# yzh503/vm-placement-migration-gym

Measured on AMD Instinct MI355X. Metric: env-steps/sec (batched) at 100-PM config, 1/2/4/8 GPUs; reward MAE vs CPU ref, higher is better.
Workload: dtype f64

## Files before the change

vm-placement-migration-gym_amd/csrc/vmp_env_common.h:

```cpp
#ifndef VMP_ENV_COMMON_H
#define VMP_ENV_COMMON_H

#include <hip/hip_runtime.h>
#include <math.h>
#include <stdint.h>

#include "vmp_dev.h"
#include "vmp_kernels.h"
#include "vmp_layout.h"
#include "vmp_np_rng.h"
#include "vmp_np_sort.h"
#include "vmp_np_sum.h"
#include "vmp_stamps.h"

namespace vmp {

struct Lds {
  EnvHdr LDSP *hdr;
  double LDSP *cpu, *mem;
  float LDSP *fcpu, *fmem;
  uint8_t LDSP *tc, *tm;
  uint16_t LDSP *ord;
  uint64_t LDSP *bc;
  int32_t LDSP *sortstk;
  uint16_t LDSP *nulls;
  uint8_t LDSP *accc, *accm;
  double LDSP *jobres;
  int32_t LDSP *arr;
  uint32_t LDSP *svc;
  uint64_t LDSP *svcst;
  uint64_t LDSP *svcfb;
  int32_t LDSP *svcinfo;
  uint8_t LDSP *ccomp, *mcomp;
  uint64_t LDSP *pdirty;
  uint32_t LDSP *evw;
  int32_t LDSP *evt;
  uint8_t LDSP *evok;
  PwLds pw;
  char LDSP *base;
};

__device__ __forceinline__ Lds make_lds(const EnvParams &p, char LDSP *base) {
  Lds L;
  L.hdr = reinterpret_cast<EnvHdr LDSP *>(base + p.off_hdr);
  L.cpu = reinterpret_cast<double LDSP *>(base + p.off_pm);
  L.mem = L.cpu + p.P;
  L.fcpu = reinterpret_cast<float LDSP *>(base + p.off_fpm);
  L.fmem = L.fcpu + p.fmem_off;
  L.tc = reinterpret_cast<uint8_t LDSP *>(base + p.off_thr);
  L.tm = L.tc + p.tm_off;
  L.ord = reinterpret_cast<uint16_t LDSP *>(base + p.off_ord);
  L.bc = reinterpret_cast<uint64_t LDSP *>(base + p.off_bits);
  L.sortstk = reinterpret_cast<int32_t LDSP *>(base + p.off_sort);
  L.nulls = reinterpret_cast<uint16_t LDSP *>(base + p.off_bits);
  L.accc = reinterpret_cast<uint8_t LDSP *>(base + p.off_acc);
  L.accm = L.accc + p.acc_cap;
  L.jobres = reinterpret_cast<double LDSP *>(base + p.off_stage);
  L.svcinfo = reinterpret_cast<int32_t LDSP *>(base + p.off_stage + kStageSvcInfo);
  L.svcfb = reinterpret_cast<uint64_t LDSP *>(base + p.off_stage + kStageSvcFb);
  L.svcst = reinterpret_cast<uint64_t LDSP *>(base + p.off_pre);
  L.svc = reinterpret_cast<uint32_t LDSP *>(base + p.off_pre + kSpecStateBytes * p.scap);
  L.arr = reinterpret_cast<int32_t LDSP *>(base + p.off_pre + kSpecDrawBytes * p.scap);
  L.pdirty = reinterpret_cast<uint64_t LDSP *>(base + p.off_pdirty);
  L.ccomp = reinterpret_cast<uint8_t LDSP *>(base + p.off_ccomp);
  L.mcomp = L.ccomp + p.ccomp_cap;
  L.evw = reinterpret_cast<uint32_t LDSP *>(base + p.off_ev);
  L.evt = reinterpret_cast<int32_t LDSP *>(L.evw + kEvCap);
  L.evok = reinterpret_cast<uint8_t LDSP *>(L.evt + kEvCap);
  L.pw.lo = reinterpret_cast<int32_t LDSP *>(base + p.off_leaf);
  L.pw.len = L.pw.lo + p.n_leaf;
  L.pw.stk = L.pw.len + p.n_leaf;
  L.pw.val = reinterpret_cast<double LDSP *>(base + p.off_leafval);
  L.base = base;
  return L;
}

struct Tables {
  double cent[128];
  float fcent[128];
  PoisConst pois[2];
};
static_assert(sizeof(Tables) == 1696 && sizeof(Tables) <= kEnvStaticLds, "k_env static LDS");

__device__ __forceinline__ int w_pl(uint32_t w) { return (int)(w & 0xFFFFu); }
constexpr int kPad = 0xFFFF;
__device__ __forceinline__ bool live(uint32_t w) { return w_pl(w) != kPad; }
__device__ __forceinline__ int w_cc(uint32_t w) { return (int)((w >> 16) & 0xFFu); }
__device__ __forceinline__ int w_cm(uint32_t w) { return (int)(w >> 24); }
__device__ __forceinline__ uint32_t w_make(int pl, int cc, int cm) {
  return (uint32_t)pl | ((uint32_t)cc << 16) | ((uint32_t)cm << 24);
}

__device__ __forceinline__ Pcg ld_pcg(const EnvHdr LDSP *h, int k) {
  Pcg r;
  r.s = U128{h->rng[k][0], h->rng[k][1]};
  r.inc = U128{h->rng[k][2], h->rng[k][3]};
  return r;
}
__device__ __forceinline__ void st_pcg(EnvHdr LDSP *h, int k, const Pcg &r) {
  if (lane_id() == 0) {
    h->rng[k][0] = r.s.hi;
    h->rng[k][1] = r.s.lo;
  }
}

__device__ __forceinline__ float fcent_of(int k) { return (float)((double)k * 0.01); }

__device__ __forceinline__ int fit_threshold(float f) {
  int k0 = (int)((1.0f - f) * 100.0f);
  k0 = k0 < 0 ? 0 : (k0 > 100 ? 100 : k0);
  const bool up = k0 < 100 && f + fcent_of(k0 + 1) <= 1.0f;
  const bool at = f + fcent_of(k0) <= 1.0f;
  return up ? k0 + 1 : (at ? k0 : k0 - 1);
}

__device__ __forceinline__ uint32_t prefix_or32(uint32_t x) {
  x |= (uint32_t)__builtin_amdgcn_update_dpp(0, (int)x, 0x111, 0xF, 0xF, false);
  x |= (uint32_t)__builtin_amdgcn_update_dpp(0, (int)x, 0x112, 0xF, 0xF, false);
  x |= (uint32_t)__builtin_amdgcn_update_dpp(0, (int)x, 0x114, 0xF, 0xF, false);
  x |= (uint32_t)__builtin_amdgcn_update_dpp(0, (int)x, 0x118, 0xF, 0xF, false);
  x |= (uint32_t)__builtin_amdgcn_update_dpp(0, (int)x, 0x142, 0xA, 0xF, false);
  x |= (uint32_t)__builtin_amdgcn_update_dpp(0, (int)x, 0x143, 0xC, 0xF, false);
  return x;
}
__device__ __forceinline__ uint64_t prefix_or64(uint64_t x) {
  return ((uint64_t)prefix_or32((uint32_t)(x >> 32)) << 32) | prefix_or32((uint32_t)x);
}

__device__ __forceinline__ uint32_t prefix_max32(uint32_t x) {
  x = max(x, (uint32_t)__builtin_amdgcn_update_dpp(0, (int)x, 0x111, 0xF, 0xF, false));
  x = max(x, (uint32_t)__builtin_amdgcn_update_dpp(0, (int)x, 0x112, 0xF, 0xF, false));
  x = max(x, (uint32_t)__builtin_amdgcn_update_dpp(0, (int)x, 0x114, 0xF, 0xF, false));
  x = max(x, (uint32_t)__builtin_amdgcn_update_dpp(0, (int)x, 0x118, 0xF, 0xF, false));
  x = max(x, (uint32_t)__builtin_amdgcn_update_dpp(0, (int)x, 0x142, 0xA, 0xF, false));
  x = max(x, (uint32_t)__builtin_amdgcn_update_dpp(0, (int)x, 0x143, 0xC, 0xF, false));
  return x;
}

__device__ __forceinline__ uint64_t readlane_u64(uint64_t x, int l) {
  const uint32_t lo = (uint32_t)__builtin_amdgcn_readlane((int)(uint32_t)x, l);
  const uint32_t hi = (uint32_t)__builtin_amdgcn_readlane((int)(uint32_t)(x >> 32), l);
  return ((uint64_t)hi << 32) | lo;
}

__device__ __forceinline__ void build_fitmax(const EnvParams &p, const Lds &L, uint32_t LDSP *M) {
  const int lane = lane_id();
  M[lane] = 0;
  M[lane + 64] = 0;
  wsync();
  for (int q = lane; q < p.P; q += 64) {
    const int tcq = (int)L.tc[q];
    if (tcq > 0) __atomic_fetch_max(&M[tcq - 1], (uint32_t)L.tm[q], __ATOMIC_RELAXED);
  }
  wsync();
  const int rlo = 63 - lane, rhi = 127 - lane;
  const bool hi_ok = rhi <= 100;
  uint32_t c1 = hi_ok ? M[rhi] : 0u, c0 = M[rlo];
  c1 = prefix_max32(c1);
  c0 = max(prefix_max32(c0), (uint32_t)__builtin_amdgcn_readlane((int)c1, 63));
  wsync();
  M[rlo] = c0;
  if (hi_ok) M[rhi] = c1;
  wsync();
}

__device__ __forceinline__ int ff_scan(const EnvParams &p, const Lds &L, int kc, int km) {
  const int lane = lane_id();
  for (int b = 0; b < p.P; b += 64) {
    const int i = b + lane;
    const bool f = i < p.P && (int)L.tc[i] - 1 >= kc && (int)L.tm[i] - 1 >= km;
    const uint64_t m = ballot(f);
    if (m) return b + __ffsll((unsigned long long)m) - 1;
  }
  return -1;
}

__device__ __forceinline__ int bf_tie(const EnvParams &p, const Lds &L, int kc, int km, int above,
                                   int eq);
__device__ __forceinline__ int bf_choose(const EnvParams &p, const Lds &L, int kc, int km) {
  const int lane = lane_id();
  const int P = p.P;
  float best = -INFINITY;
  int cnt = 0, bi = -1;
  for (int i = lane; i < P; i += 64) {
    if ((int)L.tc[i] - 1 >= kc && (int)L.tm[i] - 1 >= km) {
      const float key = L.fcpu[i] + L.fmem[i];
      if (key > best) {
        best = key;
        cnt = 1;
        bi = i;
      } else if (key == best) {
        cnt++;
      }
    }
  }
  float m = best;
#pragma unroll
  for (int o = 32; o > 0; o >>= 1) m = fmaxf(m, __shfl_xor(m, o));
  int tot = (best == m) ? cnt : 0;
#pragma unroll
  for (int o = 32; o > 0; o >>= 1) tot += __shfl_xor(tot, o);
  if (tot == 0) return -1;
  if (tot == 1) {
    const uint64_t who = ballot(best == m && cnt == 1);
    return __builtin_amdgcn_readlane(bi, __ffsll((unsigned long long)who) - 1);
  }
  int above = 0, eq = 0;
  for (int i = lane; i < P; i += 64) {
    const float key = L.fcpu[i] + L.fmem[i];
    above += key > m;
    eq += key == m;
  }
#pragma unroll
  for (int o = 32; o > 0; o >>= 1) {
    above += __shfl_xor(above, o);
    eq += __shfl_xor(eq, o);
  }
  return bf_tie(p, L, kc, km, above, eq);
}

__device__ __forceinline__ int bf_tie(const EnvParams &p, const Lds &L, int kc, int km, int above,
                                   int eq) {
  const int lane = lane_id();
  const int P = p.P;
  for (int i = lane; i < P; i += 64) L.ord[i] = (uint16_t)i;
  const int hi = P - above - 1, lo = P - above - eq;
  wsync();
  const uint8_t LDSP *tc = L.tc, *tm = L.tm;
  const int pos = wave_aqselect_top(
      KeySum{L.fcpu, L.fmem}, L.ord, P, L.sortstk, lo, hi,
      reinterpret_cast<uint16_t LDSP *>(L.sortstk + kSortStackWords),
      [=](int q) { return (int)tc[q] - 1 >= kc && (int)tm[q] - 1 >= km; });
  return pos >= 0 ? (int)L.ord[pos] : -1;
}

__device__ __forceinline__ void mark_pm(const Lds &L, int P, int q) {
  L.pdirty[q >> 6] |= 1ull << (q & 63);
  L.pdirty[(P + q) >> 6] |= 1ull << ((P + q) & 63);
}

__device__ __forceinline__ bool env_place(const Lds &L, const Tables &T, int P, int q, int kc,
                                          int km) {
  double cq = L.cpu[q], mq = L.mem[q];
  double vc = T.cent[kc], vm = T.cent[km];
  bool ok = (cq + vc <= 1) && (mq + vm <= 1);
  wsync();
  if (ok && lane_id() == 0) {
    L.cpu[q] = cq + vc;
    L.mem[q] = mq + vm;
    mark_pm(L, P, q);
  }
  wsync();
  return ok;
}

__device__ __noinline__ uint32_t svc_fallback(uint64_t LDSP *st, const uint64_t LDSP *inc,
                                              const PoisConst *c) {
  Pcg r;
  r.s = U128{st[0], st[1]};
  r.inc = U128{inc[0], inc[1]};
  const int64_t x = poisson(r, *c);
  __builtin_amdgcn_fence(__ATOMIC_SEQ_CST, "wavefront");
  __builtin_amdgcn_wave_barrier();
  if ((threadIdx.x & 63) == 0) {
    st[0] = r.s.hi;
    st[1] = r.s.lo;
  }
  __builtin_amdgcn_fence(__ATOMIC_SEQ_CST, "wavefront");
  __builtin_amdgcn_wave_barrier();
  return (uint32_t)(x + 1);
}

struct ParRng {
  U128 base, inc;
  U128 st;
  double u;
  int pos;
};
__device__ __forceinline__ U128 rl128(U128 x, int l) {
  return U128{readlane_u64(x.hi, l), readlane_u64(x.lo, l)};
}
__device__ __forceinline__ void par_fill(ParRng &g, const U128 &JA, const U128 &JM) {
  g.st = add128(mul128(JA, g.base), mul128(JM, g.inc));
  const uint64_t x = g.st.hi ^ g.st.lo;
  const unsigned rot = (unsigned)(g.st.hi >> 58);
  const uint64_t out = (x >> rot) | (x << ((64 - rot) & 63));
  g.u = (double)(out >> 11) * (1.0 / 9007199254740992.0);
  g.pos = 0;
}
__device__ __forceinline__ void par_next_chunk(ParRng &g, const U128 &JA, const U128 &JM) {
  g.base = rl128(g.st, 63);
  par_fill(g, JA, JM);
}
__device__ __forceinline__ U128 par_state(const ParRng &g) {
  return g.pos == 0 ? g.base : rl128(g.st, uni(g.pos - 1));
}

__device__ __forceinline__ int64_t par_poisson_mult(ParRng &g, double enlam, const U128 &JA,
                                                    const U128 &JM) {
  double prod = 1.0;
  int64_t X = 0;
#pragma unroll 1
  for (;;) {
    if (g.pos == 64) par_next_chunk(g, JA, JM);
    prod *= readlane_f64(g.u, uni(g.pos));
    g.pos++;
    if (prod > enlam)
      X += 1;
    else
      return X;
  }
}

struct PtrsChunk {
  uint64_t acc;
  int64_t k;
  bool valid;
};
__device__ __forceinline__ void par_ptrs_eval(const ParRng &g, const PoisConst &c, PtrsChunk &pc) {
  const int lane = lane_id();
  const int i = lane & 31;
  const double U = __shfl(g.u, 2 * i) - 0.5;
  const double V = __shfl(g.u, 2 * i + 1);
  const double us = 0.5 - fabs(U);
  const int64_t k = (int64_t)floor((2 * c.a / us + c.b) * U + c.lam + 0.43);
  bool ok;
  if ((us >= 0.07) && (V <= c.vr))
    ok = true;
  else if ((k < 0) || ((us < 0.013) && (V > us)))
    ok = false;
  else
    ok = ptrs_accept(V, us, k, c.lam, c.a, c.b, c.loglam, c.log_invalpha, c.loggam_tab, c.tab_n);
  pc.acc = ballot(ok && lane < 32);
  pc.k = k;
  pc.valid = true;
}
__device__ __forceinline__ int64_t par_poisson_ptrs(ParRng &g, const PoisConst &c, PtrsChunk &pc,
                                                    const U128 &JA, const U128 &JM) {
#pragma unroll 1
  for (;;) {
    if (g.pos == 64) {
      par_next_chunk(g, JA, JM);
      pc.valid = false;
    }
    if (!pc.valid) par_ptrs_eval(g, c, pc);
    const uint64_t m = pc.acc & (~0ull << (g.pos >> 1));
    if (m == 0) {
      g.pos = 64;
      continue;
    }
    const int i = uni(__builtin_ctzll(m));
    g.pos = 2 * i + 2;
    return (int64_t)readlane_u64((uint64_t)pc.k, i);
  }
}

__device__ __forceinline__ int64_t par_poisson(ParRng &g, const PoisConst &c, PtrsChunk &pc,
                                               const U128 &JA, const U128 &JM) {
  if (c.kind == 0) return 0;
  if (c.kind == 1) return par_poisson_mult(g, c.enlam, JA, JM);
  return par_poisson_ptrs(g, c, pc, JA, JM);
}

__device__ __forceinline__ void predraw(const EnvParams &p, const Lds &L, const Tables &T,
                                        int K, int V, const U128 &JA, const U128 &JM) {
  const int lane = lane_id();
  EnvHdr LDSP *H = L.hdr;
  ParRng g;
  PtrsChunk pc;
  pc.valid = false;
  Pcg r3 = ld_pcg(H, 2);
  g.base = r3.s;
  g.inc = r3.inc;
  par_fill(g, JA, JM);
  int64_t need = 0;
#pragma unroll 1
  for (int k = 0; k < K; k++) {
    const int64_t a = par_poisson(g, T.pois[0], pc, JA, JM);
    if (lane == 0) L.arr[k] = (int32_t)(a < 0x7fffffff ? a : 0x7fffffff);
    need += a < V ? a : V;
  }
  r3.s = par_state(g);
  st_pcg(H, 2, r3);
  Pcg r4 = ld_pcg(H, 3);
  const uint64_t hint = H->pad;
  const bool none_free = K == 1 && (hint >> 63) && ((hint >> 32) & 1u) == 0 &&
                         (uint32_t)hint > (uint32_t)H->timestep + 1u;
  const int S = none_free ? 0 : (int)(need < p.scap ? need : p.scap);
  g.base = r4.s;
  g.inc = r4.inc;
  pc.valid = false;
  if (S > 0) par_fill(g, JA, JM);
#pragma unroll 1
  for (int j = 0; j < S; j++) {
    const int64_t x = par_poisson(g, T.pois[1], pc, JA, JM);
    const U128 sj = par_state(g);
    if (lane == 0) {
      L.svc[j] = (uint32_t)(x + 1);
      L.svcst[2 * j] = sj.hi;
      L.svcst[2 * j + 1] = sj.lo;
    }
  }
  const U128 fb = S > 0 ? par_state(g) : r4.s;
  if (lane == 0) {
    L.svcfb[0] = fb.hi;
    L.svcfb[1] = fb.lo;
    L.svcinfo[0] = S;
    L.svcinfo[1] = 0;
  }
  wsync();
}

constexpr int kSrcConfig = 0, kSrcEnv = 1, kSrcTrace = 2;
template <int SRC>
__device__ __forceinline__ const PoisConst *env_pois(const EnvParams &p, int e) {
  return SRC == kSrcEnv ? p.pois + 2 * (int64_t)e : p.pois;
}

template <int SRC>
__device__ __forceinline__ uint32_t svc_take(const EnvParams &p, const Lds &L, int e) {
  const int S = L.svcinfo[0], used = L.svcinfo[1];
  uint32_t x;
  if (used < S) {
    x = L.svc[used];
  } else {
    x = svc_fallback(L.svcfb, &L.hdr->rng[3][2], env_pois<SRC>(p, e) + 1);
  }
  wsync();
  if (lane_id() == 0) L.svcinfo[1] = used + 1;
  wsync();
  return x;
}

__device__ __forceinline__ void svc_commit(const Lds &L) {
  const int S = L.svcinfo[0], used = L.svcinfo[1];
  if (used == 0) return;
  uint64_t hi, lo;
  if (used <= S) {
    hi = L.svcst[2 * (used - 1)];
    lo = L.svcst[2 * (used - 1) + 1];
  } else {
// ... 60 lines not shown
```

vm-placement-migration-gym_amd/csrc/vmp_env_wave.h:

```cpp
#ifndef VMP_ENV_WAVE_H
#define VMP_ENV_WAVE_H

#include <hip/hip_runtime.h>
#include <stdint.h>

#include "vmp_dev.h"
#include "vmp_env_common.h"
#include "vmp_kernels.h"
#include "vmp_launch_order.h"
#include "vmp_layout.h"
#include "vmp_stamps.h"

namespace vmp {

template <int VPT>
__device__ __forceinline__ int64_t heuristic_apply(const EnvParams &p, const Lds &L,
                                                   const Tables &T, uint32_t (&wa)[VPT],
                                                   int policy, int32_t *act_out,
                                                   uint8_t *valid_out, bool quiet, int qkind,
                                                   bool &fit_any STAMP_PARAMS) {
  const int lane = lane_id();
  const int P = p.P, WAIT = p.P;
  const bool bf = policy == 1;
  uint32_t pend = 0;
#pragma unroll
  for (int s = 0; s < VPT; s++)
    if (w_pl(wa[s]) == WAIT) pend |= 1u << s;
  uint32_t won = 0, bad = 0;
  int64_t n_place = 0;
  fit_any = false;
#ifdef VMP_CHECK_QUIET
  if (ballot(pend != 0)) {
#else
  if (!quiet && ballot(pend != 0)) {
#endif
    for (int i = lane; i < P; i += 64) {
      const float fcv = (float)L.cpu[i], fmv = (float)L.mem[i];
      L.fcpu[i] = fcv;
      L.fmem[i] = fmv;
      L.tc[i] = (uint8_t)(fit_threshold(fcv) + 1);
      L.tm[i] = (uint8_t)(fit_threshold(fmv) + 1);
    }
    wsync();
    STAMP(16);
    uint32_t hit = 0;
    uint32_t LDSP *M = reinterpret_cast<uint32_t LDSP *>(L.bc);
    build_fitmax(p, L, M);
#pragma unroll
    for (int s = 0; s < VPT; s++)
      hit |= (uint32_t)(((pend >> s) & 1u) && M[w_cc(wa[s])] > (uint32_t)w_cm(wa[s])) << s;
    const bool anyfit = ballot(hit != 0) != 0;
    fit_any = anyfit;
#ifdef VMP_CHECK_QUIET
    if (quiet && qkind == 1 && anyfit && lane == 0)
      __hip_atomic_fetch_add(gptr(&g_quiet_violations), 1ull, __ATOMIC_RELAXED,
                             __HIP_MEMORY_SCOPE_AGENT);
#endif
    STAMP(17);
#pragma unroll 1
    for (; anyfit;) {
      const int mine = hit ? (__builtin_ctz(hit) << 6) | lane : 2047;
      const int best = 2047 - (int)__builtin_amdgcn_readlane(
                                  (int)prefix_max32((uint32_t)(2047 - mine)), 63);
      STAMP(18);
      if (best == 2047) break;
      const int ws = best >> 6, wl = best & 63;
      uint32_t own = 0;
#pragma unroll
      for (int s = 0; s < VPT; s++)
        if (s == ws) own = wa[s];
      const uint32_t ww = rdlane(own, wl);
#pragma unroll
      for (int s = 0; s < VPT; s++)
        if (s < ws || (s == ws && lane <= wl)) pend &= ~(1u << s);
      hit &= pend;
      const int kc = w_cc(ww), km = w_cm(ww);
      const int q = bf ? bf_choose(p, L, kc, km) : ff_scan(p, L, kc, km);
      const double cq = L.cpu[q], mq = L.mem[q];
      const float fq = L.fcpu[q], fmq = L.fmem[q];
      const int tc_old = (int)L.tc[q] - 1, tm_old = (int)L.tm[q] - 1;
      const double vc = T.cent[kc], vm = T.cent[km];
      const bool ok = (cq + vc <= 1) && (mq + vm <= 1);
      const float nc = fq + T.fcent[kc];
      const float nm = fmq + T.fcent[km];
      const int t = fit_threshold(nc);
      const int tmq = bf ? fit_threshold(nm) : tm_old;
      wsync();
      if (lane == 0) {
        if (ok) {
          L.cpu[q] = cq + vc;
          L.mem[q] = mq + vm;
          mark_pm(L, P, q);
        }
        L.fcpu[q] = nc;
        L.tc[q] = (uint8_t)(t + 1);
        if (bf) {
          L.fmem[q] = nm;
          L.tm[q] = (uint8_t)(tmq + 1);
        }
      }
      wsync();
      n_place += ok;
      STAMP(20);
      if (lane == wl) {
#pragma unroll
        for (int s = 0; s < VPT; s++)
          if (s == ws) {
            won |= 1u << s;
            if (ok) wa[s] = (wa[s] & 0xFFFF0000u) | (uint32_t)q;
            else bad |= 1u << s;
          }
        if (act_out) gptr(act_out)[ws * 64 + wl] = q;
      }
      STAMP(21);
      if (t < tc_old || tmq < tm_old) {
        build_fitmax(p, L, M);
        STAMP(23);
#pragma unroll
        for (int s0 = 0; s0 < VPT; s0 += 4) {
          uint32_t mc[4];
#pragma unroll
          for (int j = 0; j < 4; j++) mc[j] = s0 + j < VPT ? M[w_cc(wa[s0 + j])] : 0u;
#pragma unroll
          for (int j = 0; j < 4; j++)
            if (s0 + j < VPT && !(mc[j] > (uint32_t)w_cm(wa[s0 + j]))) hit &= ~(1u << (s0 + j));
        }
      }
      STAMP(19);
    }
  }
#ifdef VMP_CHECK_QUIET
  if (quiet && qkind == 2 && n_place > 0 && lane == 0)
    __hip_atomic_fetch_add(gptr(&g_quiet_violations), 1ull, __ATOMIC_RELAXED,
                           __HIP_MEMORY_SCOPE_AGENT);
#endif
  if (act_out || valid_out) {
    const int ln = fresh_lane();
#pragma unroll
    for (int s = 0; s < VPT; s++) {
      const int v = s * 64 + ln;
      if (live(wa[s])) {
        if (act_out && !((won >> s) & 1u)) gptr(act_out)[v] = (int32_t)w_pl(wa[s]);
        if (valid_out) gptr(valid_out)[v] = (uint8_t)!((bad >> s) & 1u);
      }
    }
  }
  return n_place;
}

template <int VPT>
__device__ __forceinline__ void external_apply(const EnvParams &p, const Lds &L, const Tables &T,
                                               uint32_t (&wa)[VPT], const int32_t *act_row,
                                               uint8_t *valid_out, int64_t &n_place,
                                               int64_t &n_susp) {
  const int lane = lane_id();
  const int P = p.P, WAIT = p.P;
  const int32_t GLBP *ar = gptr(act_row);
  int32_t tv[VPT];
  __asm__ volatile("" ::: "memory");
#pragma unroll
  for (int s = 0; s < VPT; s++) tv[s] = ar[min(s * 64 + lane, p.V - 1)];
#pragma unroll
  for (int s = 0; s < VPT; s++) {
    const int v = s * 64 + lane;
    const bool in = live(wa[s]);
    const int c = w_pl(wa[s]);
    const int t = in ? tv[s] : c;
    const bool isplace = in && c == WAIT && t >= 0 && t < P;
    const bool issusp = in && c < P && t == WAIT;
    uint64_t evm = ballot(isplace || issusp);
    uint64_t okm = 0;
    const uint32_t me = wa[s];
#pragma unroll 1
    while (evm) {
      const int l = __ffsll((unsigned long long)evm) - 1;
      evm &= evm - 1;
      const uint32_t ew = rdlane(me, l);
      const int et = __builtin_amdgcn_readlane(t, l);
      const int ec = w_pl(ew);
      const double vc = T.cent[w_cc(ew)], vm = T.cent[w_cm(ew)];
      const int q = (ec == WAIT) ? et : ec;
      double cq = L.cpu[q], mq = L.mem[q];
      bool eok = true;
      if (ec == WAIT) {
        eok = (cq + vc <= 1) && (mq + vm <= 1);
        if (eok) {
          cq = cq + vc;
          mq = mq + vm;
        }
      } else {
        cq = cq - vc;
        mq = mq - vm;
      }
      wsync();
      if (lane == 0) {
        L.cpu[q] = cq;
        L.mem[q] = mq;
        mark_pm(L, P, q);
      }
      okm |= (uint64_t)eok << l;
      wsync();
    }
    bool ok = (t == c) || issusp;
    if (isplace) ok = (okm >> lane) & 1ull;
    n_place += __popcll(okm & ballot(isplace));
    n_susp += __popcll(ballot(issusp));
    if (ok && t != c && in) wa[s] = (wa[s] & 0xFFFF0000u) | (uint32_t)t;
    if (valid_out && in) gptr(valid_out)[v] = (uint8_t)ok;
  }
}

template <int VPT, bool LAZY, int SRC>
__device__ __forceinline__ double env_tail(const EnvParams &p, const Lds &L, const Tables &T,
                                           uint32_t (&wa)[VPT], uint32_t (&rem)[VPT],
                                           uint32_t run0, uint32_t fb, uint32_t &dirty,
                                           uint32_t *vmo, int kstep, bool ext,
                                           bool quiet_in, bool &terminated, bool &calm,
                                           bool &has_ex, int e STAMP_PARAMS) {
  const int lane = lane_id();
  const int P = p.P, WAIT = p.P, NUL = p.P + 1;
  EnvHdr LDSP *H = L.hdr;
  const uint32_t t32 = (uint32_t)H->timestep;
  int64_t n_term = 0;
#pragma unroll
  for (int s = 0; s < VPT; s++) {
    const bool running = w_pl(wa[s]) < P;
    if (running != (bool)((run0 >> s) & 1u)) {
      if (!LAZY) rem[s] = running ? rem[s] + t32 : rem[s] - t32;
      dirty |= 1u << s;
    }
    const bool term = running && (LAZY ? (bool)((fb >> s) & 1u) : (int32_t)(rem[s] - t32) <= 1);
    uint64_t it = ballot(term);
    n_term += __popcll(it);
    const uint32_t me = wa[s];
#pragma unroll 1
    while (it) {
      const int l = __ffsll((unsigned long long)it) - 1;
      it &= it - 1;
      const uint32_t ew = rdlane(me, l);
      const int q = w_pl(ew);
      const double cq = L.cpu[q] - T.cent[w_cc(ew)];
      const double mq = L.mem[q] - T.cent[w_cm(ew)];
      wsync();
      if (lane == 0) {
        L.cpu[q] = cq;
        L.mem[q] = mq;
        mark_pm(L, P, q);
      }
      wsync();
    }
    if (term) {
      wa[s] = w_make(NUL, 0, 0);
      if (!LAZY) rem[s] = 0;
      dirty |= 1u << s;
    }
  }
  if (n_term > 0 || ext)
    for (int i = lane; i < P; i += 64) {
      if (L.cpu[i] < 1e-7) L.cpu[i] = 0;
      if (L.mem[i] < 1e-7) L.mem[i] = 0;
    }
  STAMP(2);
  const uint64_t ph = H->pad;
  const bool no_null = kstep == 0 && (ph >> 63) && !((ph >> 32) & 1u) && n_term == 0;
  int n_null = 0;
  if (!no_null) {
#pragma unroll
    for (int s = 0; s < VPT; s++) {
      const int v = s * 64 + lane;
      const bool isnull = w_pl(wa[s]) == NUL;
      const uint64_t nm = ballot(isnull);
      if (isnull) L.nulls[n_null + below(nm, lane)] = (uint16_t)v;
      n_null += __popcll(nm);
    }
  }
  const int64_t arrivals = L.arr[kstep];
  const int64_t k = arrivals < n_null ? arrivals : n_null;
  wsync();
  if (k > 0) {
    Pcg r1 = ld_pcg(H, 0), r2 = ld_pcg(H, 1);
    const uint64_t GLBP *req = nullptr;
    if constexpr (SRC == kSrcTrace) req = gptr(env_trace(p, e).req) + L.svcfb[0];
#pragma unroll 1
    for (int j = 0; j < k; j++) {
      int cc, cm;
      uint32_t rr;
      if constexpr (SRC == kSrcTrace) {
        if ((j & 63) == 0 && (j | kstep) != 0) {
          wsync();
          L.svcst[lane] = j + lane < k ? req[j + lane] : 0ull;
          wsync();
        }
        const uint64_t rq = L.svcst[j & 63];
        cc = rq_cc(rq);
        cm = rq_cm(rq);
        rr = rq_rt(rq);
      } else {
        cc = (int)rint((p.seq_lo + p.seq_range * next_double(r1)) * 100.0);
        cm = (int)rint((p.seq_lo + p.seq_range * next_double(r2)) * 100.0);
        rr = svc_take<SRC>(p, L, e);
      }
      const int v = L.nulls[j];
      if (lane == (v & 63)) {
#pragma unroll
        for (int s = 0; s < VPT; s++)
          if (s == (v >> 6)) {
            wa[s] = w_make(WAIT, cc, cm);
            if (LAZY) {
              ST_NT(vmo + vm_slot_idx(v), wa[s]);
              ST_NT(vmo + vm_time_idx(v), rr);
              dirty &= ~(1u << s);
            } else {
              rem[s] = rr;
              dirty |= 1u << s;
            }
          }
      }
      if (lane == 0) {
        L.accc[j] = (uint8_t)cc;
        L.accm[j] = (uint8_t)cm;
      }
    }
    if constexpr (SRC != kSrcTrace) {
      st_pcg(H, 0, r1);
      st_pcg(H, 1, r2);
    }
  }
  wsync();
  STAMP(3);
  const bool kl = p.reward == 2;
  int n_ex = 0, n_w = 0;
  const bool same_vms = p.reward == 0 && quiet_in && n_term == 0 && k == 0;
  if (!same_vms) {
#pragma unroll
    for (int s = 0; s < VPT; s++) {
      const int c = w_pl(wa[s]);
      const bool ex = c <= WAIT;
      const uint64_t em = ballot(ex);
      if (kl && ex) {
        const int rk = n_ex + below(em, lane);
        L.ccomp[rk] = (uint8_t)w_cc(wa[s]);
        L.mcomp[rk] = (uint8_t)w_cm(wa[s]);
      }
      n_ex += __popcll(em);
      n_w += __popcll(ballot(c == WAIT));
    }
  }
  if (!same_vms) has_ex = n_ex > 0;
  wsync();
  STAMP(11);
  double LDSP *res = L.jobres;
  const double *cent = T.cent;
  {
#pragma unroll 1
    for (int j = (k > 0 ? 0 : 2); j < (kl ? 4 : 2); j++) {
      const uint8_t LDSP *src = (j == 0) ? L.accc : (j == 1) ? L.accm : ((j & 1) ? L.mcomp : L.ccomp);
      const int n = j < 2 ? (int)k : n_ex;
      const double r = wave_pw_sum(n, [=](int i) { return cent[src[i]]; }, L.pw);
      wsync();
      if (lane == 0) res[j] = r;
      wsync();
    }
  }
  if (p.reward >= 1) {
    const int jend = p.reward == 2 ? 8 : 6;
#pragma unroll 1
    for (int j = 4; j < jend; j++) {
      const double LDSP *src = (j & 1) ? L.mem : L.cpu;
      const double mean = j < 6 ? 0.0 : res[j - 2] / (double)P;
      const bool sq = j >= 6;
      const double r = wave_pw_sum(P, [=](int i) {
        const double x = src[i];
        const double d = x - mean;
        return sq ? d * d : x;
      }, L.pw);
      wsync();
      if (lane == 0) res[j] = r;
      wsync();
    }
  }
  if (p.reward == 2) {
#pragma unroll 1
    for (int j = 8; j < 10; j++) {
      const uint8_t LDSP *src = (j & 1) ? L.mcomp : L.ccomp;
      const double mean = res[j - 6] / (double)n_ex;
      const double r = wave_pw_sum(n_ex, [=](int i) {
        const double d = cent[src[i]] - mean;
        return d * d;
      }, L.pw);
      wsync();
      if (lane == 0) res[j] = r;
      wsync();
    }
  }
  STAMP(12);
  const double wr = same_vms ? H->waiting_ratio : n_ex > 0 ? (double)n_w / (double)n_ex : 0.0;
  if (!kl) res[2] = res[3] = 0.0;
  double tcm = res[2] / (double)P;
  if (p.cap_target_util && tcm > 1) tcm = 1.0;
  double tmm = res[3] / (double)P;
  if (p.cap_target_util && tmm > 1) tmm = 1.0;
  double reward = 0.0;
  if (has_ex) {
    if (p.reward == 2) {
      double cv = res[6] / (double)P, mv = res[7] / (double)P;
      if (cv == 0) cv = 1e-6;
      if (mv == 0) mv = 1e-6;
      double tcv = res[8] / (double)n_ex, tmv = res[9] / (double)n_ex;
      if (tcv == 0) tcv = 1e-6;
      if (tmv == 0) tmv = 1e-6;
      reward = (tcm == 0 || tmm == 0)
                   ? 0.0
                   : kl_reward(tcm, tmm, tcv, tmv, res[4] / (double)P, res[5] / (double)P, cv, mv);
    } else if (p.reward == 1) {
      reward = p.beta * res[4] + (1 - p.beta) * res[5];
    } else {
      reward = -wr;
    }
  }
  STAMP(4);
  const int64_t ts = H->timestep;
  terminated = ts >= p.limit;
  calm = n_term == 0 && k == 0;
  (void)n_ex;
  wsync();
  if (lane == 0) {
    H->timestep = ts + 1;
    H->total_requests += arrivals;
    H->served += n_term;
    H->dropped += arrivals - k;
    if constexpr (SRC == kSrcTrace) L.svcfb[0] += (uint64_t)arrivals;
    H->waiting_ratio = wr;
    if (kl) {
      H->tcm = tcm;
      H->tmm = tmm;
    }
    if (k > 0) {
      H->total_cpu_req = H->total_cpu_req + res[0];
      H->total_mem_req = H->total_mem_req + res[1];
    }
  }
  wsync();
  return reward;
}

template <int VPT>
__device__ __forceinline__ void write_obs(const EnvParams &p, const Lds &L, const Tables &T,
                                          const uint32_t (&wa)[VPT], float *obs) {
  const int lane = fresh_lane();
  const int V = p.V, P = p.P;
#pragma unroll
  for (int s = 0; s < VPT; s++) {
    const int v = s * 64 + lane;
    if (live(wa[s])) {
      ST_NT(obs + v, (float)w_pl(wa[s]));
      ST_NT(obs + V + v, T.fcent[w_cc(wa[s])]);
      ST_NT(obs + 2 * V + v, T.fcent[w_cm(wa[s])]);
    }
  }
  for (int i = lane; i < P; i += 64) {
    ST_NT(obs + 3 * V + i, (float)L.cpu[i]);
    ST_NT(obs + 3 * V + P + i, (float)L.mem[i]);
  }
}

template <int VPT>
__device__ __forceinline__ void write_mask(const EnvParams &p, const Lds &L, const Tables &T,
                                           const uint32_t (&wa)[VPT], uint32_t *bits) {
  const int lane = fresh_lane();
  const int P = p.P, A = p.A, W = p.W32, WAIT = p.P, NUL = p.P + 1;
#pragma unroll
  for (int s = 0; s < VPT; s++) {
    const int v = s * 64 + lane;
    const bool in = live(wa[s]);
    const int c = in ? w_pl(wa[s]) : NUL;
    const double vc = T.cent[w_cc(wa[s])], vm = T.cent[w_cm(wa[s])];
    const bool waiting = in && c == WAIT;
    const bool anyw = ballot(waiting) != 0;
#pragma unroll 1
    for (int w = 0; w < W; w++) {
      uint32_t word = 0xFFFFFFFFu;
      const int a0 = w * 32;
      if (c >= a0 && c < a0 + 32 && c < A) word &= ~(1u << (c - a0));
      if (c < P && WAIT >= a0 && WAIT < a0 + 32) word &= ~(1u << (WAIT - a0));
      if (anyw) {
        const int hi = min(a0 + 32, P);
#pragma unroll 1
        for (int q = a0; q < hi; q++) {
          const bool fit = (L.cpu[q] + vc <= 1) && (L.mem[q] + vm <= 1);
          if (waiting && fit) word &= ~(1u << (q - a0));
        }
      }
      if (in) bits[(int64_t)v * W + w] = word;
    }
  }
}

__device__ __forceinline__ uint8_t *lo_flags(const EnvParams &p, int parity) {
  return reinterpret_cast<uint8_t *>(p.hdr + p.N) + (int64_t)parity * lo_flag_bytes(p.N);
}
__device__ __forceinline__ int lo_swap_env(const EnvParams &p, int q, int &fidx) {
  const uint32_t w = (uint32_t)p.pad0;
  fidx = -1;
  if (lo_mode(w) == kLoIdleLast) {
    const int C = lo_chunks(p.N), T = lo_T(w), nr = lo_nr(w);
    int r = q / C;
    const int c = q - r * C;
    if (lo_in_tail(r, T, nr)) {
      const int lane = lane_id();
      const uint8_t GLBP *line = gptr(lo_flags(p, lo_parity(w))) + (int64_t)c * kLoChunk;
      const bool in = lane < 2 * T;
      const uint8_t f = in ? line[lo_lane_rank(lane, T, nr)] : (uint8_t)0;
      const uint32_t busy = (uint32_t)ballot(in && f != 0);
      r = uni(lo_partner(busy, T, nr, lo_parity(w), r));
      q = r * C + c;
    }
    fidx = c * kLoChunk + r;
  }
  return q;
}
__device__ __forceinline__ void lo_store_flag(const EnvParams &p, int fidx, uint64_t ph, int64_t t) {
  if (fidx < 0) return;
  const uint32_t nf = (uint32_t)ph;
  const bool q1 = (ph >> 62) & 1u, q2 = (ph >> 60) & 1u;
  const bool idle = (ph >> 63) && q1 != q2 && (ph & 0x0FFFFFFF00000000ull) == 0 && nf != 0u &&
                    (int32_t)(nf - (uint32_t)t) > 1;
  gptr(lo_flags(p, lo_parity((uint32_t)p.pad0) ^ 1))[fidx] = (uint8_t)!idle;
}

__device__ __forceinline__ bool idle_step(const EnvParams &p, const StepOut &o, const Lds &L) {
#ifdef VMP_CHECK_QUIET
  return false;
#else
  const uint64_t ph = L.hdr->pad;
  const uint32_t t32 = (uint32_t)L.hdr->timestep;
  const uint32_t nf = (uint32_t)ph;
  const bool q1 = (ph >> 62) & 1u, q2 = (ph >> 60) & 1u;
  const bool idle = o.k_steps == 1 && p.reward == 0 && !o.act_out && !o.valid && !o.mask_bits &&
                    2 * p.P <= 256 && (ph >> 63) && q1 != q2 &&
                    (ph & 0x0FFFFFFF00000000ull) == 0 && nf != 0u && (int32_t)(nf - t32) > 1;
  return uni((int)idle) != 0;
#endif
}

template <int VPT>
__device__ __forceinline__ void idle_body(const EnvParams &p, const StepOut &o, const Lds &L,
                                          const float LDSP *fcent, int e,
                                          const uint32_t (&wa)[VPT], int fidx) {
  const int lane = lane_id();
  const int V = p.V;
  EnvHdr LDSP *H = L.hdr;
  const int64_t a = L.arr[0];
  const uint64_t ph = H->pad;
  const int64_t ts = H->timestep;
  const bool term = ts >= p.limit;
  if (lane == 0) {
    if (o.reward) gptr(o.reward)[e] = ((ph >> 61) & 1u) ? -H->waiting_ratio : 0.0;
    if (o.done) gptr(o.done)[e] = (uint8_t)term;
    if (o.done_count) gptr(o.done_count)[e] += (int64_t)term;
  }
  if (o.obs) {
    float *obs = o.obs + (int64_t)e * p.D;
#pragma unroll
    for (int s = 0; s < VPT; s++) {
      const int v = s * 64 + lane;
      if (live(wa[s])) {
        ST_NT(obs + v, (float)w_pl(wa[s]));
        ST_NT(obs + V + v, fcent[w_cc(wa[s])]);
        ST_NT(obs + 2 * V + v, fcent[w_cm(wa[s])]);
      }
    }
    for (int i = lane; i < 2 * p.P; i += 64) ST_NT(obs + 3 * V + i, (float)L.cpu[i]);
  }
  wsync();
  if (lane == 0) {
    H->timestep = ts + 1;
    H->total_requests += a;
    H->dropped += a;
    lo_store_flag(p, fidx, ph, ts + 1);
  }
  wsync();
  if (lane < 32)
    gptr(reinterpret_cast<uint64_t *>(p.hdr + e))[lane] = reinterpret_cast<uint64_t LDSP *>(H)[lane];
}

template <int VPT, bool ONE, bool EXT, int SRC>
__device__ __forceinline__ void env_body(const EnvParams &p, const StepOut &o) {
  extern __shared__ __align__(16) char lds[];
  __shared__ Tables T;
#ifdef VMP_STAMPS
  const uint64_t t_start = __builtin_amdgcn_s_memtime();
  const uint64_t rt_start = __builtin_amdgcn_s_memrealtime();
#endif
  const int lane = lane_id();
  const int wid = threadIdx.x >> 6;
  int fidx = -1;
  int e_raw = uni(blockIdx.x * kEnvWavesPerBlock + wid);
  if constexpr (ONE) e_raw = uni(lo_position((uint32_t)p.pad0, p.N, e_raw));
  int e = e_raw < p.N ? e_raw : p.N - 1;
  char LDSP *base = (char LDSP *)lds + wid * p.lds_wave_bytes;
  const Lds L = make_lds(p, base);
  const int V = p.V, P = p.P;
  __builtin_amdgcn_s_setprio(2);
  uint64_t hv = gptr(reinterpret_cast<const uint64_t *>(p.hdr + e))[lane & 31];
  if constexpr (ONE && !EXT && SRC != kSrcTrace) {
    const int e2 = uni(lo_swap_env(p, e, fidx));
    if (e2 != e) {
      e = e_raw = e2;
      hv = gptr(reinterpret_cast<const uint64_t *>(p.hdr + e))[lane & 31];
    }
  }
  static_assert(kEnvWavesPerBlock == 1, "Tables::pois holds one env's Poisson constants");
  constexpr int kPoisWords = (int)(2 * sizeof(PoisConst) / 4);
  uint32_t pw = 0;
  if constexpr (SRC != kSrcTrace)
    pw = gptr(reinterpret_cast<const uint32_t *>(env_pois<SRC>(p, e)))[threadIdx.x % kPoisWords];
  TraceDesc td{nullptr, nullptr, 0, 0};
  if constexpr (SRC == kSrcTrace) td = env_trace(p, e);
  U128 JA{0, 0}, JM{0, 0};
  if (SRC != kSrcTrace && o.k_steps > 0) {
    const uint64_t GLBP *jt = gptr(p.jump + 4 * lane);
    JA = U128{jt[0], jt[1]};
    JM = U128{jt[2], jt[3]};
  }
  const double *pm = p.pm + (int64_t)e * 2 * P;
  const int n_pm = 2 * P;
  double pv[4];
#pragma unroll
  for (int j = 0; j < 4; j++) pv[j] = pm[min(j * 64 + lane, n_pm - 1)];
  __asm__ volatile("" ::: "memory");
  const uint32_t GLBP *vlo = gptr(p.vmw + (int64_t)e * vm_pitch(V));
  uint32_t wa[VPT], rem[VPT];
#pragma unroll
  for (int s = 0; s < VPT; s++) {
    const int v = s * 64 + lane;
    const uint32_t x = vlo[vw_row(s, lane)];
    wa[s] = v < V ? x : (uint32_t)kPad;
    if (ONE) {
      rem[s] = 0;
    } else {
      const uint32_t y = vlo[vw_row(s, lane) + 64];
      rem[s] = v < V ? y : 0u;
    }
  }
  __asm__ volatile("" ::: "memory");
  __builtin_amdgcn_s_setprio(0);
  for (int i = threadIdx.x; i < 128; i += blockDim.x) {
    T.cent[i] = (double)i / 100.0;
    T.fcent[i] = (float)((double)i / 100.0);
  }
  if (SRC != kSrcTrace && threadIdx.x < kPoisWords)
    reinterpret_cast<uint32_t *>(T.pois)[threadIdx.x] = pw;
  __syncthreads();
  if (e_raw >= p.N) return;
  if (lane < 32) reinterpret_cast<uint64_t LDSP *>(L.hdr)[lane] = hv;
  wsync();
#ifdef VMP_STAMPS
  const uint64_t t_loaded = __builtin_amdgcn_s_memtime();
#endif
  if (EXT) {
#pragma unroll
    for (int j = 0; j < 4; j++)
      if (j * 64 + lane < n_pm) L.cpu[j * 64 + lane] = pv[j];
  }
  if constexpr (SRC == kSrcTrace) {
    if (o.k_steps > 0) trace_preload(L, td, o.k_steps);
  } else {
    if (o.k_steps > 0) predraw(p, L, T, o.k_steps, V, JA, JM);
  }
#ifdef VMP_STAMPS
  const uint64_t t_drawn = __builtin_amdgcn_s_memtime();
#endif
  if (!EXT) {
#pragma unroll
    for (int j = 0; j < 4; j++)
      if (j * 64 + lane < n_pm) L.cpu[j * 64 + lane] = pv[j];
  }
  for (int i = 256 + lane; i < n_pm; i += 64) L.cpu[i] = pm[i];
  for (int i = lane; i < (n_pm + 63) / 64; i += 64) L.pdirty[i] = 0;
  wsync();
#ifdef VMP_STAMPS
  __shared__ uint64_t st_lds[kEnvWavesPerBlock * kStamps];
#endif
  STAMP_DECL_AT((uint64_t LDSP *)st_lds + wid * kStamps)
#ifdef VMP_STAMPS
  if (lane == 0) {
    st_acc[13] = t_loaded - t_start;
    st_acc[14] = t_drawn - t_loaded;
    st_acc[15] = st_prev - t_drawn;
  }
#endif
  if constexpr (ONE && !EXT && SRC != kSrcTrace) {
  if (idle_step(p, o, L)) {
    idle_body<VPT>(p, o, L, (const float LDSP *)T.fcent, e, wa, fidx);
#ifdef VMP_STAMPS
    if (p.stamps && lane == 0) stamp_idle(p.stamps + (int64_t)e * kStamps, t_start, rt_start);
#endif
    return;
  }
  }
  bool term = false;
  int64_t ndone = 0;
  uint32_t dirty = 0;
  uint32_t fb = 0;
  uint32_t hiv[VPT];
  uint32_t nf = 0u;
  bool want_nf = false;
  bool skip_time = false;
  uint32_t nf_carry = 0u;
  if (ONE && !EXT) {
#ifndef VMP_CHECK_QUIET
    const uint64_t ph = L.hdr->pad;
    nf_carry = (uint32_t)ph;
    const bool skip_h = ((ph >> 62) & 1u) || (((ph >> 60) & 1u) && !o.act_out && !o.valid);
    skip_time = skip_h && (ph >> 63) && ((ph >> 32) & 1u) == 0u && nf_carry != 0u &&
                (int32_t)(nf_carry - (uint32_t)L.hdr->timestep) > 1;
#endif
    const uint32_t GLBP *hb = vlo + 64 + (skip_time ? 0 : lane);
    const int hs = skip_time ? 0 : 128;
#pragma unroll
    for (int s = 0; s < VPT; s++) hiv[s] = hb[s * hs];
    __asm__ volatile("" ::: "memory");
  }
  uint32_t *vmo = p.vmw + (int64_t)e * vm_pitch(V);
  const int k_steps = ONE ? 1 : o.k_steps;
  int qkind = EXT ? 0 : (((L.hdr->pad >> 62) & 1u) ? 1 : (((L.hdr->pad >> 60) & 1u) ? 2 : 0));
  bool has_ex = (L.hdr->pad >> 61) & 1u;
#pragma unroll 1
  for (int k = 0; k < k_steps; k++) {
    const bool last = k == k_steps - 1;
    uint8_t *valid_row = (last && o.valid) ? o.valid + (int64_t)e * V : nullptr;
    int32_t *act_row = (last && o.act_out) ? o.act_out + (int64_t)e * V : nullptr;
    int64_t n_place = 0, n_susp = 0;
    uint32_t run0 = 0;
#pragma unroll
    for (int s = 0; s < VPT; s++) run0 |= (uint32_t)(w_pl(wa[s]) < P) << s;
    bool fit_any = false;
    const bool quiet = qkind == 1 || (qkind == 2 && !act_row && !valid_row);
    if (!EXT)
      n_place = heuristic_apply<VPT>(p, L, T, wa, o.policy, act_row, valid_row, quiet, qkind,
                                     fit_any STAMP_ARGS);
    else {
      external_apply<VPT>(p, L, T, wa, o.actions + (int64_t)e * V, valid_row, n_place, n_susp);
      if (ONE) {
        const int ln = fresh_lane();
#pragma unroll
        for (int s = 0; s < VPT; s++) hiv[s] = vlo[vw_row(s, ln) + 64];
      }
    }
    STAMP(1);
    if (ONE) {
      const uint32_t t32 = (uint32_t)L.hdr->timestep;
      const uint64_t ph = L.hdr->pad;
      want_nf = !((ph >> 63) && ((ph >> 32) & 1u));
      nf = want_nf ? 0xFFFFFFFFu : 0u;
      if (skip_time) {
        nf = nf_carry;
      } else {
#pragma unroll
      for (int s = 0; s < VPT; s++) {
        const bool was_run = (run0 >> s) & 1u;
        const bool f = was_run ? (int32_t)(hiv[s] - t32) <= 1 : hiv[s] <= 1u;
        fb |= (uint32_t)f << s;
      }
      }
      if (want_nf && !skip_time) {
#pragma unroll
        for (int s = 0; s < VPT; s++) {
          const bool was_run = (run0 >> s) & 1u;
          const bool f = (fb >> s) & 1u;
          if (w_pl(wa[s]) < P && !f) nf = min(nf, was_run ? hiv[s] : hiv[s] + t32);
        }
      }
    }
    wsync();
    if (lane == 0) {
      L.hdr->place_action += n_place;
      L.hdr->suspend_action += n_susp;
    }
    wsync();
    bool calm = false;
    const double r = env_tail<VPT, ONE, SRC>(p, L, T, wa, rem, run0, fb, dirty, vmo, k, EXT, quiet,
                                        term, calm, has_ex, e STAMP_ARGS);
    qkind = (EXT || !calm) ? 0 : quiet ? qkind : (!fit_any ? 1 : (n_place == 0 ? 2 : 0));
    if (o.reward && lane == 0) gptr(o.reward)[(int64_t)k * p.N + e] = r;
    ndone += term;
  }
  if (SRC != kSrcTrace && o.k_steps > 0) svc_commit(make_lds(p, opaque_base(base)));
  if (!EXT && o.k_steps == 0 && o.policy >= 0 && o.act_out) {
    uint32_t wt[VPT];
#pragma unroll
    for (int s = 0; s < VPT; s++) wt[s] = wa[s];
    bool fit_any;
    heuristic_apply<VPT>(p, L, T, wt, o.policy, o.act_out + (int64_t)e * V, nullptr, qkind == 1,
                         qkind, fit_any STAMP_ARGS);
  }
  STAMP(0);
  if (o.obs) write_obs<VPT>(p, L, T, wa, o.obs + (int64_t)e * p.D);
  if (o.mask_bits) write_mask<VPT>(p, L, T, wa, o.mask_bits + (int64_t)e * V * p.W32);
  STAMP(5);
  if (o.k_steps > 0) {
    if (o.done && lane == 0) gptr(o.done)[e] = (uint8_t)term;
    if (o.done_count && lane == 0) gptr(o.done_count)[e] += ndone;
    const uint32_t t32 = (uint32_t)(L.hdr->timestep - 1);
    const int ln = fresh_lane();
#pragma unroll
    for (int s = 0; s < VPT; s++) {
      if (live(wa[s]) && ((dirty >> s) & 1u)) {
        const int iw = (s << 7) + ln;
        if (!ONE) {
          ST_NT(vmo + iw, wa[s]);
          ST_NT(vmo + iw + 64, rem[s]);
        } else if (w_pl(wa[s]) == P + 1) {
          ST_NT(vmo + iw, wa[s]);
          ST_NT(vmo + iw + 64, 0u);
        } else {
          uint32_t GLBP *w32 = gptr(vmo);
          w32[iw] = wa[s];
          __hip_atomic_fetch_add(w32 + iw + 64, w_pl(wa[s]) < P ? t32 : 0u - t32,
                                 __ATOMIC_RELAXED, __HIP_MEMORY_SCOPE_AGENT);
        }
      }
    }
    double *pmo = p.pm + (int64_t)e * 2 * P;
    for (int i = lane, j = 0; i < 2 * P; i += 64, j++)
      if ((L.pdirty[j] >> lane) & 1ull) ST_NT(pmo + i, (double)L.cpu[i]);
    {
      uint64_t hint = 0;
      if (ONE) {
        bool anynull = false;
#pragma unroll
        for (int s = 0; s < VPT; s++) anynull |= w_pl(wa[s]) == P + 1;
        uint32_t m = nf;
        const bool nn = ballot(anynull) != 0;
        if (!nn && want_nf) {
#pragma unroll
          for (int o = 32; o > 0; o >>= 1) m = min(m, (uint32_t)__shfl_xor((int)m, o));
        }
        hint = (1ull << 63) | ((uint64_t)nn << 32) | m;
      }
      hint |= ((uint64_t)(qkind == 1) << 62) | ((uint64_t)(qkind == 2) << 60) |
              ((uint64_t)has_ex << 61);
      wsync();
      if (lane == 0) {
        L.hdr->pad = hint;
        if constexpr (ONE && !EXT && SRC != kSrcTrace) lo_store_flag(p, fidx, hint, L.hdr->timestep);
      }
      wsync();
    }
    if (lane < 32)
      gptr(reinterpret_cast<uint64_t *>(p.hdr + e))[lane] = reinterpret_cast<uint64_t LDSP *>(L.hdr)[lane];
  }
  STAMP(6);
#ifdef VMP_STAMPS
  if (lane == 0) {
    st_acc[7] = (__builtin_amdgcn_s_memrealtime() - rt_start) * 1000;
    st_acc[9] = __builtin_amdgcn_s_memtime() - t_start;
  }
#endif
  STAMP_FLUSH();
}

template <int VPT, bool ONE, bool WL>
__global__ __launch_bounds__(64 * kEnvWavesPerBlock, ONE ? VMP_WAVES_PER_EU_ONE : VMP_WAVES_PER_EU) void k_env(EnvParams p, StepOut o) {
  env_body<VPT, ONE, false, WL ? kSrcEnv : kSrcConfig>(p, o);
}
template <int VPT, bool WL>
__global__ __launch_bounds__(64 * kEnvWavesPerBlock, VPT == 1 ? 4 : VMP_WAVES_PER_EU_ONE) void k_env_ext(EnvParams p, StepOut o) {
  env_body<VPT, true, true, WL ? kSrcEnv : kSrcConfig>(p, o);
}
template <int VPT, bool ONE>
__global__ __launch_bounds__(64 * kEnvWavesPerBlock, ONE ? VMP_WAVES_PER_EU_ONE : VMP_WAVES_PER_EU) void k_env_tr(EnvParams p, StepOut o) {
  env_body<VPT, ONE, false, kSrcTrace>(p, o);
}
template <int VPT>
__global__ __launch_bounds__(64 * kEnvWavesPerBlock, VPT == 1 ? 4 : VMP_WAVES_PER_EU_ONE) void k_env_ext_tr(EnvParams p, StepOut o) {
  env_body<VPT, true, true, kSrcTrace>(p, o);
}

#ifdef VMP_ENV_TR
template __global__ void k_env_ext_tr<1>(EnvParams, StepOut);
template __global__ void k_env_ext_tr<2>(EnvParams, StepOut);
template __global__ void k_env_ext_tr<4>(EnvParams, StepOut);
template __global__ void k_env_ext_tr<8>(EnvParams, StepOut);
template __global__ void k_env_ext_tr<16>(EnvParams, StepOut);
template __global__ void k_env_tr<1, false>(EnvParams, StepOut);
template __global__ void k_env_tr<1, true>(EnvParams, StepOut);
template __global__ void k_env_tr<2, false>(EnvParams, StepOut);
template __global__ void k_env_tr<2, true>(EnvParams, StepOut);
template __global__ void k_env_tr<4, false>(EnvParams, StepOut);
template __global__ void k_env_tr<4, true>(EnvParams, StepOut);
template __global__ void k_env_tr<8, false>(EnvParams, StepOut);
template __global__ void k_env_tr<8, true>(EnvParams, StepOut);
template __global__ void k_env_tr<16, false>(EnvParams, StepOut);
template __global__ void k_env_tr<16, true>(EnvParams, StepOut);
#else
#ifndef VMP_ENV_WL
#define VMP_ENV_WL false
#endif
template __global__ void k_env_ext<1, VMP_ENV_WL>(EnvParams, StepOut);
template __global__ void k_env_ext<2, VMP_ENV_WL>(EnvParams, StepOut);
template __global__ void k_env_ext<4, VMP_ENV_WL>(EnvParams, StepOut);
template __global__ void k_env_ext<8, VMP_ENV_WL>(EnvParams, StepOut);
template __global__ void k_env_ext<16, VMP_ENV_WL>(EnvParams, StepOut);
template __global__ void k_env<1, false, VMP_ENV_WL>(EnvParams, StepOut);
template __global__ void k_env<1, true, VMP_ENV_WL>(EnvParams, StepOut);
template __global__ void k_env<2, false, VMP_ENV_WL>(EnvParams, StepOut);
template __global__ void k_env<2, true, VMP_ENV_WL>(EnvParams, StepOut);
template __global__ void k_env<4, false, VMP_ENV_WL>(EnvParams, StepOut);
template __global__ void k_env<4, true, VMP_ENV_WL>(EnvParams, StepOut);
template __global__ void k_env<8, false, VMP_ENV_WL>(EnvParams, StepOut);
template __global__ void k_env<8, true, VMP_ENV_WL>(EnvParams, StepOut);
template __global__ void k_env<16, false, VMP_ENV_WL>(EnvParams, StepOut);
template __global__ void k_env<16, true, VMP_ENV_WL>(EnvParams, StepOut);
#endif

}

#endif
```

Before: 273.0 million.

## Track waiting/null VM counts incrementally instead of rescanning VM slots each step

Counts waiting VMs once up front with a DPP wave reduction, then updates the wait and remaining-null counters incrementally from the place, suspend and arrival counts instead of rescanning every VM slot per step. In the lazy path it skips the termination loop when no running VM has a finish bit, and skips the per-VM dirty writeback when nothing is dirty. The null-presence hint now comes from the tracked counter rather than a scan. This adds state carried across steps in the k-loop, which risks the counters drifting from the true state if any transition is missed.

```diff
diff --git a/vm-placement-migration-gym_amd/csrc/vmp_env_common.h b/vm-placement-migration-gym_amd/csrc/vmp_env_common.h
--- a/vm-placement-migration-gym_amd/csrc/vmp_env_common.h
+++ b/vm-placement-migration-gym_amd/csrc/vmp_env_common.h
@@ -137,6 +137,16 @@
   return x;
 }
 
+__device__ __forceinline__ uint32_t wave_sum32(uint32_t x) {
+  x += (uint32_t)__builtin_amdgcn_update_dpp(0, (int)x, 0x111, 0xF, 0xF, false);
+  x += (uint32_t)__builtin_amdgcn_update_dpp(0, (int)x, 0x112, 0xF, 0xF, false);
+  x += (uint32_t)__builtin_amdgcn_update_dpp(0, (int)x, 0x114, 0xF, 0xF, false);
+  x += (uint32_t)__builtin_amdgcn_update_dpp(0, (int)x, 0x118, 0xF, 0xF, false);
+  x += (uint32_t)__builtin_amdgcn_update_dpp(0, (int)x, 0x142, 0xA, 0xF, false);
+  x += (uint32_t)__builtin_amdgcn_update_dpp(0, (int)x, 0x143, 0xC, 0xF, false);
+  return (uint32_t)__builtin_amdgcn_readlane((int)x, 63);
+}
+
 __device__ __forceinline__ uint64_t readlane_u64(uint64_t x, int l) {
   const uint32_t lo = (uint32_t)__builtin_amdgcn_readlane((int)(uint32_t)x, l);
   const uint32_t hi = (uint32_t)__builtin_amdgcn_readlane((int)(uint32_t)(x >> 32), l);
diff --git a/vm-placement-migration-gym_amd/csrc/vmp_env_wave.h b/vm-placement-migration-gym_amd/csrc/vmp_env_wave.h
--- a/vm-placement-migration-gym_amd/csrc/vmp_env_wave.h
+++ b/vm-placement-migration-gym_amd/csrc/vmp_env_wave.h
@@ -18,7 +18,8 @@
                                                    const Tables &T, uint32_t (&wa)[VPT],
                                                    int policy, int32_t *act_out,
                                                    uint8_t *valid_out, bool quiet, int qkind,
-                                                   bool &fit_any STAMP_PARAMS) {
+                                                   bool &fit_any, bool count_wait,
+                                                   int &n_wait STAMP_PARAMS) {
   const int lane = lane_id();
   const int P = p.P, WAIT = p.P;
   const bool bf = policy == 1;
@@ -26,6 +27,7 @@
 #pragma unroll
   for (int s = 0; s < VPT; s++)
     if (w_pl(wa[s]) == WAIT) pend |= 1u << s;
+  if (count_wait) n_wait = (int)wave_sum32((uint32_t)__popc(pend));
   uint32_t won = 0, bad = 0;
   int64_t n_place = 0;
   fit_any = false;
@@ -152,9 +154,10 @@
 __device__ __forceinline__ void external_apply(const EnvParams &p, const Lds &L, const Tables &T,
                                                uint32_t (&wa)[VPT], const int32_t *act_row,
                                                uint8_t *valid_out, int64_t &n_place,
-                                               int64_t &n_susp) {
+                                               int64_t &n_susp, int &n_wait) {
   const int lane = lane_id();
   const int P = p.P, WAIT = p.P;
+  int n_wait0 = 0;
   const int32_t GLBP *ar = gptr(act_row);
   int32_t tv[VPT];
   __asm__ volatile("" ::: "memory");
@@ -166,6 +169,7 @@
     const bool in = live(wa[s]);
     const int c = w_pl(wa[s]);
     const int t = in ? tv[s] : c;
+    n_wait0 += __popcll(ballot(c == WAIT));
     const bool isplace = in && c == WAIT && t >= 0 && t < P;
     const bool issusp = in && c < P && t == WAIT;
     uint64_t evm = ballot(isplace || issusp);
@@ -208,25 +212,39 @@
     if (ok && t != c && in) wa[s] = (wa[s] & 0xFFFF0000u) | (uint32_t)t;
     if (valid_out && in) gptr(valid_out)[v] = (uint8_t)ok;
   }
-}
-
-template <int VPT, bool LAZY, int SRC>
+  n_wait = n_wait0;
+}
+
+template <int VPT, bool LAZY, int SRC, bool EXTK>
 __device__ __forceinline__ double env_tail(const EnvParams &p, const Lds &L, const Tables &T,
                                            uint32_t (&wa)[VPT], uint32_t (&rem)[VPT],
                                            uint32_t run0, uint32_t fb, uint32_t &dirty,
-                                           uint32_t *vmo, int kstep, bool ext,
-                                           bool quiet_in, bool &terminated, bool &calm,
-                                           bool &has_ex, int e STAMP_PARAMS) {
+                                           uint32_t *vmo, int kstep,
+                                           bool quiet_in, int64_t n_place, int64_t n_susp,
+                                           int &n_w, int &null_left, bool &terminated,
+                                           bool &calm, bool &has_ex, int e STAMP_PARAMS) {
   const int lane = lane_id();
   const int P = p.P, WAIT = p.P, NUL = p.P + 1;
   EnvHdr LDSP *H = L.hdr;
   const uint32_t t32 = (uint32_t)H->timestep;
   int64_t n_term = 0;
+  uint32_t run1 = run0;
+  bool any_fin = true;
+  if (LAZY) {
+    if (n_place != 0 || n_susp != 0) {
+      run1 = 0;
+#pragma unroll
+      for (int s = 0; s < VPT; s++) run1 |= (uint32_t)(w_pl(wa[s]) < P) << s;
+      dirty |= run1 ^ run0;
+    }
+    any_fin = ballot((fb & run1) != 0u) != 0;
+  }
+  if (any_fin) {
 #pragma unroll
   for (int s = 0; s < VPT; s++) {
-    const bool running = w_pl(wa[s]) < P;
-    if (running != (bool)((run0 >> s) & 1u)) {
-      if (!LAZY) rem[s] = running ? rem[s] + t32 : rem[s] - t32;
+    const bool running = LAZY ? (bool)((run1 >> s) & 1u) : w_pl(wa[s]) < P;
+    if (!LAZY && running != (bool)((run0 >> s) & 1u)) {
+      rem[s] = running ? rem[s] + t32 : rem[s] - t32;
       dirty |= 1u << s;
     }
     const bool term = running && (LAZY ? (bool)((fb >> s) & 1u) : (int32_t)(rem[s] - t32) <= 1);
@@ -255,7 +273,8 @@
       dirty |= 1u << s;
     }
   }
-  if (n_term > 0 || ext)
+  }
+  if (n_term > 0 || n_susp > 0)
     for (int i = lane; i < P; i += 64) {
       if (L.cpu[i] < 1e-7) L.cpu[i] = 0;
       if (L.mem[i] < 1e-7) L.mem[i] = 0;
@@ -329,22 +348,25 @@
   wsync();
   STAMP(3);
   const bool kl = p.reward == 2;
-  int n_ex = 0, n_w = 0;
+  null_left = n_null - (int)k;
+  n_w += (int)n_susp - (int)n_place + (int)k;
+  int n_ex = p.V - null_left;
+  __builtin_assume(n_ex >= 0 && n_ex <= VPT * 64);
   const bool same_vms = p.reward == 0 && quiet_in && n_term == 0 && k == 0;
-  if (!same_vms) {
+  if (EXTK || kl) {
+    int off = 0;
 #pragma unroll
     for (int s = 0; s < VPT; s++) {
-      const int c = w_pl(wa[s]);
-      const bool ex = c <= WAIT;
+      const bool ex = w_pl(wa[s]) <= WAIT;
       const uint64_t em = ballot(ex);
       if (kl && ex) {
-        const int rk = n_ex + below(em, lane);
+        const int rk = off + below(em, lane);
         L.ccomp[rk] = (uint8_t)w_cc(wa[s]);
         L.mcomp[rk] = (uint8_t)w_cm(wa[s]);
       }
-      n_ex += __popcll(em);
-      n_w += __popcll(ballot(c == WAIT));
-    }
+      off += __popcll(em);
+    }
+    if (EXTK) n_ex = off;
   }
   if (!same_vms) has_ex = n_ex > 0;
   wsync();
@@ -726,6 +748,7 @@
   const int k_steps = ONE ? 1 : o.k_steps;
   int qkind = EXT ? 0 : (((L.hdr->pad >> 62) & 1u) ? 1 : (((L.hdr->pad >> 60) & 1u) ? 2 : 0));
   bool has_ex = (L.hdr->pad >> 61) & 1u;
+  int n_w = 0, null_left = 0;
 #pragma unroll 1
   for (int k = 0; k < k_steps; k++) {
     const bool last = k == k_steps - 1;
@@ -739,9 +762,10 @@
     const bool quiet = qkind == 1 || (qkind == 2 && !act_row && !valid_row);
     if (!EXT)
       n_place = heuristic_apply<VPT>(p, L, T, wa, o.policy, act_row, valid_row, quiet, qkind,
-                                     fit_any STAMP_ARGS);
+                                     fit_any, k == 0, n_w STAMP_ARGS);
     else {
-      external_apply<VPT>(p, L, T, wa, o.actions + (int64_t)e * V, valid_row, n_place, n_susp);
+      external_apply<VPT>(p, L, T, wa, o.actions + (int64_t)e * V, valid_row, n_place, n_susp,
+                          n_w);
       if (ONE) {
         const int ln = fresh_lane();
 #pragma unroll
@@ -780,8 +804,9 @@
     }
     wsync();
     bool calm = false;
-    const double r = env_tail<VPT, ONE, SRC>(p, L, T, wa, rem, run0, fb, dirty, vmo, k, EXT, quiet,
-                                        term, calm, has_ex, e STAMP_ARGS);
+    const double r = env_tail<VPT, ONE, SRC, EXT>(p, L, T, wa, rem, run0, fb, dirty, vmo, k, quiet,
+                                        n_place, n_susp, n_w, null_left, term, calm, has_ex,
+                                        e STAMP_ARGS);
     qkind = (EXT || !calm) ? 0 : quiet ? qkind : (!fit_any ? 1 : (n_place == 0 ? 2 : 0));
     if (o.reward && lane == 0) gptr(o.reward)[(int64_t)k * p.N + e] = r;
     ndone += term;
@@ -793,7 +818,7 @@
     for (int s = 0; s < VPT; s++) wt[s] = wa[s];
     bool fit_any;
     heuristic_apply<VPT>(p, L, T, wt, o.policy, o.act_out + (int64_t)e * V, nullptr, qkind == 1,
-                         qkind, fit_any STAMP_ARGS);
+                         qkind, fit_any, false, n_w STAMP_ARGS);
   }
   STAMP(0);
   if (o.obs) write_obs<VPT>(p, L, T, wa, o.obs + (int64_t)e * p.D);
@@ -804,6 +829,7 @@
     if (o.done_count && lane == 0) gptr(o.done_count)[e] += ndone;
     const uint32_t t32 = (uint32_t)(L.hdr->timestep - 1);
     const int ln = fresh_lane();
+    if (!ONE || ballot(dirty != 0u) != 0) {
 #pragma unroll
     for (int s = 0; s < VPT; s++) {
       if (live(wa[s]) && ((dirty >> s) & 1u)) {
@@ -822,17 +848,21 @@
         }
       }
     }
+    }
     double *pmo = p.pm + (int64_t)e * 2 * P;
     for (int i = lane, j = 0; i < 2 * P; i += 64, j++)
       if ((L.pdirty[j] >> lane) & 1ull) ST_NT(pmo + i, (double)L.cpu[i]);
     {
       uint64_t hint = 0;
       if (ONE) {
-        bool anynull = false;
-#pragma unroll
-        for (int s = 0; s < VPT; s++) anynull |= w_pl(wa[s]) == P + 1;
         uint32_t m = nf;
-        const bool nn = ballot(anynull) != 0;
+        bool nn = null_left > 0;
+        if (EXT) {
+          bool anynull = false;
+#pragma unroll
+          for (int s = 0; s < VPT; s++) anynull |= w_pl(wa[s]) == P + 1;
+          nn = ballot(anynull) != 0;
+        }
         if (!nn && want_nf) {
 #pragma unroll
           for (int o = 32; o > 0; o >>= 1) m = min(m, (uint32_t)__shfl_xor((int)m, o));
```

New measurement: 282.0 million (median of 6 runs). 1.03x the previous value.
